# algbio/founderblockgraphs

Hardware: AMD Instinct MI355X
Metric: MSA columns segmented/sec (higher is better)
Workload: dtype u32

## Files before the change

founderblockgraphs_amd/csrc/ctx.hip:

```cpp
#include "fbg_internal.h"
#include <chrono>
#include <stdarg.h>
#include <stdio.h>
#include <ctype.h>
#include <string.h>
#include <algorithm>
#include <atomic>
#include <thread>
#include <vector>

static std::string g_global_err;

int fbg_fail(fbg_ctx *ctx, int code, const char *fmt, ...)
{
    char buf[1024];
    va_list ap;
    va_start(ap, fmt);
    vsnprintf(buf, sizeof(buf), fmt, ap);
    va_end(ap);
    if (ctx) ctx->err = buf; else g_global_err = buf;
    return code;
}

int fbg_reserve(fbg_ctx *ctx, DevBuf &b, size_t bytes, std::vector<DevBuf *> *owner, bool accounted)
// ... 167 lines not shown
    {"gapped_rank", &FbgOptions::gapped_rank},
    {"part_tricks_off", &FbgOptions::part_tricks_off},
    {"msd_sample_bins", &FbgOptions::msd_sample_bins},
    {"msd_min_force", &FbgOptions::msd_min_force},
    {"msd_probe", &FbgOptions::msd_probe},
    {"msd_xcd", &FbgOptions::msd_xcd},
    {"rank_no_lean", &FbgOptions::rank_no_lean},
    {"no_stream_upload", &FbgOptions::no_stream_upload},
    {"span_scan", &FbgOptions::span_scan},
    {"span_key_flags", &FbgOptions::span_key_flags},
    {"span_slow_split", &FbgOptions::span_slow_split},
    {"poison", &FbgOptions::poison},
    {"dpw_matrix", &FbgOptions::dpw_matrix},
    {"dp_chain1", &FbgOptions::dp_chain1},
    {"msd_ext", &FbgOptions::msd_ext},
};

struct InfoKey { const char *name; int64_t (*get)(const fbg_ctx &); };
static const InfoKey g_info_keys[] = {
    {"grs_threshold", [](const fbg_ctx &c) -> int64_t { return c.grs_t; }},
    {"grs_redone", [](const fbg_ctx &c) -> int64_t { return (int64_t)c.grs_redone; }},
    {"dp_kind", [](const fbg_ctx &c) -> int64_t { return c.dp_kind; }},
    {"msd_decline", [](const fbg_ctx &c) -> int64_t { return c.diag.msd_decline; }},
    {"pass1_ahead", [](const fbg_ctx &c) -> int64_t { return c.diag.pass1_ahead; }},
    {"ext_pairs", [](const fbg_ctx &c) -> int64_t { return c.diag.ext_pairs; }},
    {"text_pairs", [](const fbg_ctx &c) -> int64_t { return c.diag.text_pairs; }},
    {"rank_lean_used", [](const fbg_ctx &c) -> int64_t { return c.diag.rank_lean_used; }},
    {"rank_lean_launched", [](const fbg_ctx &c) -> int64_t { return c.diag.rank_lean_launched; }},
    {"pairs_rb", [](const fbg_ctx &c) -> int64_t { return c.diag.pairs_rb; }},
    {"key_b", [](const fbg_ctx &c) -> int64_t { return c.key_b; }},
    {"key_K", [](const fbg_ctx &c) -> int64_t { return c.key_K; }},
    {"key_packed", [](const fbg_ctx &c) -> int64_t { return c.key_packed; }},
    {"key_compact", [](const fbg_ctx &c) -> int64_t { return c.key_compact; }},
    {"alloc_calls", [](const fbg_ctx &c) -> int64_t { return (int64_t)c.alloc_calls; }},
    {"alloc_us", [](const fbg_ctx &c) -> int64_t { return (int64_t)c.alloc_us; }},
    {"span_decline", [](const fbg_ctx &c) -> int64_t { return c.diag.sp_decline; }},
    {"span_key_flags_used", [](const fbg_ctx &c) -> int64_t { return c.ix.index_valid && c.ix.spanned() && c.ix.sp_key_flags_sorted; }},
    {"span_scan_used", [](const fbg_ctx &c) -> int64_t { return c.ix.index_valid && c.ix.spanned(); }},
    {"span_scan_work", [](const fbg_ctx &c) -> int64_t { return (int64_t)c.sp_work; }},
    {"span_groups", [](const fbg_ctx &c) -> int64_t { return (int64_t)c.sp_G; }},
    {"span_odd_groups", [](const fbg_ctx &c) -> int64_t { return (int64_t)c.sp_n_odd[0] + c.sp_n_odd[1] + c.sp_n_odd[2] + c.sp_n_odd[3]; }},
    {"span_irregular", [](const fbg_ctx &c) -> int64_t { return (int64_t)c.sp_n_irr; }},
// ... 519 lines not shown
```

founderblockgraphs_amd/csrc/fbg_internal.h:

```cpp
#pragma once
#include <cstring>
#include <cstdlib>
#include <hip/hip_runtime.h>
#include <stdint.h>
#include <string>
#include <vector>
#include "../../include/fbg_hip.h"

#define FBG_WAVE 64

struct DevBuf {
    void *p = nullptr;
    size_t cap = 0;
    bool listed = false;
    template <class T> T *as() const { return reinterpret_cast<T *>(p); }
};

struct Stager {
    void *base = nullptr;
    size_t slot_bytes = 0;
    int nslots = 0;
    hipEvent_t *ev = nullptr;
    hipStream_t stream = nullptr;
};

struct StageTimer {
    hipEvent_t start = nullptr, stop = nullptr;
    bool recorded = false;
    int launches = 0;
};

struct FbgOptions {
    int64_t no_ranked = 0, no_packed = 0, force_wide = 0, full_keys = 0, no_msd_sort = 0, msd_min = -1, bp_min = -1,
            record_scatter = 0, lcp_text = 0, no_aux_stream = 0, rank_no_threshold = 0, dp_literal = 0, dp_wave = 0,
            dp_safe_window = 0, dp_tile = 0, pure_scan = 0, gapped_rank = 0, part_tricks_off = 0, msd_sample_bins = 0, msd_min_force = 0, msd_probe = 0, msd_xcd = -1, rank_no_lean = 0, no_stream_upload = 0,
            span_scan = 0, span_key_flags = 0, span_slow_split = 0, poison = 0, dpw_matrix = 0, dp_chain1 = 0, msd_ext = 1;
};

enum class IndexKind { none, record, ranked, gapped, span };

struct IndexState {
    bool index_valid = false;
    IndexKind kind = IndexKind::none;
    bool ranked() const { return kind == IndexKind::ranked; }
    bool granked() const { return kind == IndexKind::gapped || kind == IndexKind::span; }
    bool spanned() const { return kind == IndexKind::span; }
    uint32_t *sa_ptr = nullptr;
    uint64_t *rk_keys = nullptr;
    int rk_b = 0, rk_key_bits = 0, rk_K = 0;
    int rk_layout = 0, rk_pb = 0;
    bool grs_flagged = false;
// ... 4 lines not shown
    uint32_t n_exc = 0;
    bool part_active = false;
    bool gpart = false;
    int part = 0, nparts = 1;
    uint64_t part_count = 0;
    uint64_t part_T = 0;
    uint32_t part_gmin = 0;
};

struct BuildDiag {
    int64_t msd_decline = -1;
    int pass1_ahead = 0;
    int64_t ext_pairs = -1, text_pairs = -1;
    int rank_lean_launched = 0;
    int rank_lean_used = 0;
    int pairs_rb = -1;
    int sp_decline = 0;
};

struct SortExtras {
    const uint64_t *ebits = nullptr;
    const uint32_t *payload = nullptr;
    bool key_flags = false;
};

struct MsdPlan;
struct fbg_ctx {
    int device = 0;
    FbgOptions opt;
    std::string err;
// ... 17 lines not shown
    bool allow_wide = false;
    uint32_t mp = 0;
    DevBuf text;
    DevBuf pos, tot;
    DevBuf segtab;
    DevBuf colT;
    DevBuf gwin_rows;

    const uint8_t *up_host = nullptr;
    hipStream_t up_stream = nullptr;
    hipEvent_t up_ev[9] = {};
    bool pre_pass1 = false;
    uint64_t pre_symbols[4] = {0, 0, 0, 0};
    MsdPlan *pre_plan = nullptr;
    uint64_t pre_tiles = 0;

    IndexState ix;
    BuildDiag diag;
    int key_b = -1, key_K = -1, key_packed = -1, key_compact = -1;
    int dp_kind = -1;
    bool grs_skip = false;
    bool cells_built = false;
    uint64_t held_bytes = 0;
    uint64_t alloc_calls = 0, alloc_us = 0;
    std::vector<DevBuf *> bufs;

    DevBuf prow;
    DevBuf igrow;
    DevBuf rec;
    DevBuf xlist;
// ... 40 lines not shown
    do {                             \
        int rc_ = (expr);            \
        if (rc_ != FBG_OK) return rc_; \
    } while (0)

int fbg_reserve(fbg_ctx *ctx, DevBuf &b, size_t bytes, std::vector<DevBuf *> *owner, bool accounted);
inline int fbg_reserve(fbg_ctx *ctx, DevBuf &b, size_t bytes) { return fbg_reserve(ctx, b, bytes, &ctx->bufs, true); }
void fbg_release(fbg_ctx *ctx, DevBuf &b);
void fbg_release_all(fbg_ctx *ctx, std::vector<DevBuf *> &bufs);
void fbg_index_reset(fbg_ctx *ctx);
int fbg_upload(fbg_ctx *ctx, void *d_dst, const void *h_src, size_t bytes);
int fbg_download(fbg_ctx *ctx, void *h_dst, const void *d_src, size_t bytes);
int fbg_stage_begin(fbg_ctx *ctx, int stage);
int fbg_stage_end(fbg_ctx *ctx, int stage, int launches);

#define FBG_SLOTS_PAIRS 0
#define FBG_SLOTS_PACKED 1
#define FBG_SLOTS_WIDE 2
struct KeyGeom {
    int b = 0, K = 0, key_bits = 0;
    bool compact = false, packed = false;
    bool wide = false;
    int pb = 0;
    const uint8_t *d_code = nullptr;
};

inline void fbg_remember_slots(fbg_ctx *ctx, uint64_t *keys, uint32_t *vals, int layout, const KeyGeom &g)
{
    ctx->ix.rk_keys = keys; ctx->ix.sa_ptr = vals; ctx->ix.rk_layout = layout; ctx->ix.rk_pb = g.pb;
    ctx->ix.rk_b = g.b; ctx->ix.rk_key_bits = g.key_bits; ctx->ix.rk_K = g.K;
// ... 25 lines not shown
bool fbg_span_key_flags(fbg_ctx *ctx, KeyGeom &g);
int fbg_span_prepare(fbg_ctx *ctx, const KeyGeom &g, const SortExtras &x, int *launches);
int fbg_span_try(fbg_ctx *ctx, uint64_t *keys, uint32_t *vals, const KeyGeom &g, int *done);
int fbg_span_rescan(fbg_ctx *ctx, int disable_tricks, int *ok);
int fbg_build_cell_tables(fbg_ctx *ctx);
int fbg_key_setup(fbg_ctx *ctx, bool compact, KeyGeom *g, int *launches);
int fbg_rank_part_classify(fbg_ctx *ctx, uint64_t *keys, uint32_t *vals, uint64_t count, const KeyGeom &g, int pre_ok,
                           uint8_t *d_blob, int *ok);
int fbg_rank_part_runs(fbg_ctx *ctx, const uint8_t *d_blobs, uint32_t *d_gmax, int *ok);
int fbg_rank_part_unfilled(fbg_ctx *ctx, uint64_t *unfilled);
int fbg_rank_part_rescan(fbg_ctx *ctx);
int fbg_part_sort(fbg_ctx *ctx, int part, int nparts, uint8_t *d_blob, int *ok);
int fbg_msd_sort(fbg_ctx *ctx, const KeyGeom &g, uint64_t **sorted, int *ok, int *launches);
int fbg_msd_pre_begin(fbg_ctx *ctx, int *ok);
int fbg_msd_pre_pass1(fbg_ctx *ctx, uint64_t avail);
bool fbg_msd_pre_geom(fbg_ctx *ctx, KeyGeom *g);
void fbg_msd_pre_free(fbg_ctx *ctx);
int fbg_msd_sort_part(fbg_ctx *ctx, const KeyGeom &g, uint64_t lo, uint64_t hi, int nohi, int nparts, uint64_t out_offset,
                      uint64_t *count, int *ok, int *launches);
int fbg_sample_sort_pairs(fbg_ctx *ctx, const KeyGeom &g, const SortExtras &x, int *ok, int *launches);
int fbg_scan_columns(fbg_ctx *ctx, uint64_t x0, uint64_t x1, int mode, int disable_tricks,
                     uint64_t *d_out);
int fbg_dp_minmax(fbg_ctx *ctx, const uint64_t *d_f, uint64_t n, uint64_t *d_boundaries,
                  uint64_t *count_out, uint64_t *d_mml, uint64_t *d_bt);
int fbg_dp_repeatfree(fbg_ctx *ctx, const uint64_t *d_v, uint64_t n, uint64_t *d_s,
                      uint64_t *d_prev, uint64_t *d_boundaries, uint64_t *count_out);
int fbg_gapped_v_from_f(fbg_ctx *ctx, const uint64_t *d_f, uint64_t n, uint64_t *d_v);
int fbg_dp_gapped(fbg_ctx *ctx, const uint64_t *d_v, uint64_t n, uint64_t *d_s, uint64_t *d_prev,
                  uint64_t *d_boundaries, uint64_t *count_out);

// ... 11 lines not shown
```

founderblockgraphs_amd/csrc/msd_keys.h:

```cpp
#pragma once
#include <stdint.h>

#define MSD_SEP 0x80
#define MSD_ITEMS 8

template <int TILE>
__device__ __forceinline__ void msd_fetch_raw(const uint8_t *__restrict__ T, uint64_t N, uint64_t base, uint64_t &raw, uint64_t &raw2)
{
    const uint64_t p = base + threadIdx.x * 8;
    raw = p < N + 56 ? *reinterpret_cast<const uint64_t *>(T + p) : 0ull;
    raw2 = 0;
    if (threadIdx.x < 8) {
        const uint64_t q = base + TILE + threadIdx.x * 8;
        raw2 = q < N + 56 ? *reinterpret_cast<const uint64_t *>(T + q) : 0ull;
    }
}
template <int TILE, bool FULL = false>
__device__ __forceinline__ void msd_store_tile(uint8_t *tile, const uint8_t *cd, uint64_t N, uint64_t base, uint64_t raw, uint64_t raw2)
{
    const int k8 = threadIdx.x * 8;
    const uint64_t p = base + k8;
    uint64_t codes = 0;
#pragma unroll
    for (int j = 0; j < 8; j++) {
// ... 9 lines not shown
        for (int j = 0; j < 8; j++) {
            const uint32_t c = (FULL || q + j < N) ? cd[(raw2 >> (8 * j)) & 255u] : (uint32_t)MSD_SEP;
            codes2 |= (uint64_t)c << (8 * j);
        }
        *reinterpret_cast<uint64_t *>(tile + kk) = codes2;
    }
}
template <int TILE, bool FULL = false>
__device__ __forceinline__ void msd_load_tile(uint8_t *tile, const uint8_t *cd, const uint8_t *__restrict__ T, uint64_t N, uint64_t base)
{
    uint64_t raw, raw2;
    msd_fetch_raw<TILE>(T, N, base, raw, raw2);
    msd_store_tile<TILE, FULL>(tile, cd, N, base, raw, raw2);
}

__device__ __forceinline__ void msd_build_keys(const uint8_t *tile, int t0, int b, int K, uint64_t *w)
{
    bool slow = true;
    if (b == 2 && K + MSD_ITEMS - 1 <= 32) {
        uint64_t P = 0, any = 0;
#pragma unroll
        for (int q = 0; q < 4; q++) {
            const uint64_t x = *reinterpret_cast<const uint64_t *>(tile + t0 + 8 * q);
            any |= x;
            const uint32_t lo = (uint32_t)x & 0x03030303u, hi = (uint32_t)(x >> 32) & 0x03030303u;
            const uint32_t g = (((lo * 0x40100401u) >> 24) << 8) | ((hi * 0x40100401u) >> 24);
            P |= (uint64_t)g << (48 - 16 * q);
        }
        slow = (any & 0x8080808080808080ull) != 0;
#pragma unroll
// ... 31 lines not shown
```

founderblockgraphs_amd/csrc/msd_sort.hip:

```cpp
#include "fbg_internal.h"
#include "msd_keys.h"
#include <rocprim/rocprim.hpp>
#include <algorithm>
#include <cmath>

#define MSD_DIG 9
#define MSD_NB (1 << MSD_DIG)
#define MSD_THREADS 1024
#define MSD_TILE (MSD_THREADS * MSD_ITEMS)
#define MSD_TILE_BITS 13
#define MSD_XSYM 4
#define MSD_XBITS 8
static_assert(MSD_TILE == 1 << MSD_TILE_BITS, "tile size");
#define MSD_FN_THREADS 512
#define MSD_FN_CAP 4096
#define MSD_FN_ITEMS (MSD_FN_CAP / MSD_FN_THREADS)
#define MSD_FN_BITS 11
#define MSD_FN_BINS (1 << MSD_FN_BITS)
#define MSD_BIG_THREADS 1024
#define MSD_BIG_CAP 16384
#define MSD_ARENA (1u << 20)

struct MsdArgs {
    const uint8_t *T;
    uint64_t N;
    const uint8_t *code;
    int b, K, pb, kb;
    int xb;
    uint8_t *ext;
    uint64_t *buf1;
    uint64_t cap1;
    int xs;
    uint64_t segcap;
    unsigned long long *count1;
    const uint32_t *tile_start;
    uint64_t tile0;
    uint32_t tiles2, tiles2_x;
    uint64_t *buf2;
    uint32_t *count2;
    const unsigned long long *off;
    uint64_t *out;
// ... 13 lines not shown
#pragma unroll
    for (int d = 1; d < 64; d <<= 1) { const uint32_t o = __shfl_up(inc, d, 64); if ((int)lane >= d) inc += o; }
    if (lane == 63) wsum[wv] = inc;
    __syncthreads();
    uint32_t pre = 0;
    for (uint32_t q = 0; q < wv; q++) pre += wsum[q];
    if (threadIdx.x < MSD_NB) {
        loff[threadIdx.x] = pre + inc - c;
        unsigned long long g = 0;
        if (c) g = wide_cursor ? atomicAdd(cursor_d, (unsigned long long)c) : (unsigned long long)atomicAdd(cursor32_d, c);
        gdelta[threadIdx.x] = (uint32_t)g - (pre + inc - c);
    }
    __syncthreads();
}

template <bool FULL, bool EXT>
__device__ __forceinline__ void msd_pack_split_body(const MsdArgs &a, uint64_t *buf, const uint8_t *cd, uint32_t *cnt, uint32_t *loff, uint32_t *gdelta,
                                                    uint32_t *wsum)
{
    uint8_t *tile = reinterpret_cast<uint8_t *>(buf);
    const int b = a.b, K = a.K;
    const uint64_t base = ((uint64_t)blockIdx.x + a.tile0) * MSD_TILE;
    msd_load_tile<MSD_TILE, FULL>(tile, cd, a.T, a.N, base);
    __syncthreads();
    const int t0 = threadIdx.x * MSD_ITEMS;
    uint64_t w[MSD_ITEMS];
    msd_build_keys(tile, t0, b, EXT ? K + MSD_XSYM : K, w);
    __syncthreads();
    uint32_t rk[MSD_ITEMS];
    const int dshift = a.kb + (EXT ? MSD_XBITS : 0) - MSD_DIG;
#pragma unroll
    for (int i = 0; i < MSD_ITEMS; i++) {
        const uint64_t p = base + t0 + i;
        const bool ok = FULL || p < a.N;
        rk[i] = ok ? atomicAdd(&cnt[(uint32_t)(w[i] >> dshift)], 1u) : 0xffffffffu;
        w[i] = EXT ? (w[i] << MSD_TILE_BITS) | (uint64_t)(t0 + i) : (w[i] << a.pb) | p;
    }
    __syncthreads();
// ... 11 lines not shown
#pragma unroll
    for (int r = 0; r < MSD_ITEMS; r++) {
        const uint32_t j = threadIdx.x + r * MSD_THREADS;
        if (FULL || j < have) {
            uint64_t x = buf[j];
            const uint32_t d = (uint32_t)(x >> wshift);
            if (EXT) x = (((x >> MSD_TILE_BITS) & kmask) << a.pb) | (base + (x & (MSD_TILE - 1)));
            const uint32_t at = j + gdelta[d];
            if (at < a.segcap) obase[(uint64_t)d * a.cap1 + at] = x;
            else over = true;
        }
    }
    if (over) atomicOr(a.flag, 2ull);
}

template <bool EXT>
__global__ __launch_bounds__(MSD_THREADS) void k_msd_pack_split(MsdArgs a)
{
    __shared__ uint64_t buf[MSD_TILE];
    __shared__ uint8_t cd[256];
    __shared__ uint32_t cnt[MSD_NB], loff[MSD_NB];
    __shared__ uint32_t gdelta[MSD_NB];
    __shared__ uint32_t wsum[MSD_THREADS / 64];
    if (threadIdx.x < 256) cd[threadIdx.x] = a.code[threadIdx.x];
    if (threadIdx.x < MSD_NB) cnt[threadIdx.x] = 0;
    __syncthreads();
    msd_pack_split_body<false, EXT>(a, buf, cd, cnt, loff, gdelta, wsum);
}

static void msd_launch_pass1(const MsdArgs &a, unsigned tiles, hipStream_t st)
{
    if (a.xb) hipLaunchKernelGGL(k_msd_pack_split<true>, dim3(tiles), dim3(MSD_THREADS), 0, st, a);
    else hipLaunchKernelGGL(k_msd_pack_split<false>, dim3(tiles), dim3(MSD_THREADS), 0, st, a);
}

__global__ __launch_bounds__(1024) void k_msd_tiles(const unsigned long long *__restrict__ count1, uint64_t segcap, uint32_t nseg,
                                                    uint32_t *__restrict__ tile_start, unsigned long long *__restrict__ flag)
{
    __shared__ uint32_t wsum[16];
    const uint32_t lane = threadIdx.x & 63, wv = threadIdx.x >> 6;
    uint32_t t[4], tot = 0;
#pragma unroll
    for (int q = 0; q < 4; q++) {
        const uint32_t s = threadIdx.x * 4 + q;
        t[q] = 0;
        if (s < nseg) {
            const unsigned long long c = count1[s] < segcap ? count1[s] : segcap;
            if (count1[s] > segcap) atomicOr(flag, 4ull);
// ... 310 lines not shown
    const uint64_t cap1 = (N / MSD_NB + N / (4 * MSD_NB) + 65536) & ~127ull;
    const uint64_t nsub = (uint64_t)MSD_NB * MSD_NB;
    if (N / nsub + N / (32 * nsub) + 64 > MSD_FN_CAP) return FBG_OK;
    FBG_TRY(fbg_reserve(ctx, ctx->keysA, (size_t)MSD_NB * cap1 * 8));
    FBG_TRY(fbg_reserve(ctx, ctx->keysB, (size_t)nsub * MSD_FN_CAP * 8));
    const uint32_t nseg = MSD_NB * (uint32_t)xs;
    FBG_TRY(fbg_reserve(ctx, ctx->dp_a, (size_t)nseg * 8 + ((size_t)nseg + 1) * 4 + 64));
    FBG_TRY(fbg_reserve(ctx, ctx->dp_b, nsub * 4));
    FBG_TRY(fbg_reserve(ctx, ctx->dp_c, (nsub + 1) * 8));
    FBG_TRY(fbg_reserve(ctx, ctx->dp_d, (size_t)MSD_ARENA * 4 * 2));
    FBG_TRY(fbg_reserve(ctx, ctx->dp_e, (size_t)MSD_ARENA * 8 * 2));
    const bool ext = ctx->opt.msd_ext != 0 && g.b == 2 && g.key_bits + MSD_XBITS + MSD_TILE_BITS <= 64 && g.K + MSD_XSYM + MSD_ITEMS - 1 <= 64;
    if (ext) FBG_TRY(fbg_reserve(ctx, ctx->msd_ext, (size_t)N));
    unsigned long long *flag = ctx->scalars.as<unsigned long long>() + 100;
    MsdArgs &a = p->a;
    a.T = ctx->text.as<uint8_t>(); a.N = N; a.code = g.d_code; a.b = g.b; a.K = g.K; a.pb = g.pb; a.kb = g.key_bits;
    a.xb = ext ? MSD_XBITS : 0; a.ext = ext ? ctx->msd_ext.as<uint8_t>() : nullptr;
    a.buf1 = ctx->keysA.as<uint64_t>(); a.cap1 = cap1; a.xs = xs; a.segcap = cap1 / xs;
    a.tile0 = 0; a.tiles2 = 0; a.tiles2_x = 0;
    a.count1 = ctx->dp_a.as<unsigned long long>();
    p->tile_start = reinterpret_cast<uint32_t *>(ctx->dp_a.as<uint8_t>() + (size_t)nseg * 8);
    a.tile_start = p->tile_start;
    a.buf2 = ctx->keysB.as<uint64_t>();
    a.count2 = ctx->dp_b.as<uint32_t>();
    p->off = ctx->dp_c.as<unsigned long long>();
    a.off = p->off;
    a.out = ctx->keysA.as<uint64_t>();
    a.flag = flag;
    a.arena_sb = ctx->dp_d.as<uint32_t>(); a.arena_w = ctx->dp_e.as<uint64_t>(); a.arena_count = flag + 1; a.arena_cap = MSD_ARENA;
    p->g = g; p->nsub = nsub; p->nseg = nseg; p->rest = rest; p->fbits = fbits; p->xcd = xcd; p->flag = flag;
    FBG_HIP_TRY(ctx, hipMemsetAsync(flag, 0, 16, st));
// ... 21 lines not shown
    return FBG_OK;
}

int fbg_msd_pre_pass1(fbg_ctx *ctx, uint64_t avail)
{
    MsdArgs a = ctx->pre_plan->a;
    const uint64_t N = a.N;
    const uint64_t upto = avail >= N ? (N + MSD_TILE - 1) / MSD_TILE : (avail >= 64 ? (avail - 64) / MSD_TILE : 0);
    if (upto <= ctx->pre_tiles) return FBG_OK;
    a.tile0 = ctx->pre_tiles;
    msd_launch_pass1(a, (unsigned)(upto - ctx->pre_tiles), ctx->stream);
    ctx->pre_tiles = upto;
    return FBG_OK;
}

void fbg_msd_pre_free(fbg_ctx *ctx)
{
    delete ctx->pre_plan;
    ctx->pre_plan = nullptr;
}

static bool msd_plan_current(const fbg_ctx *ctx, const MsdPlan &p)
{
    const MsdArgs &a = p.a;
    return a.T == ctx->text.p && a.code == ctx->small.as<uint8_t>() + 2048 && a.buf1 == ctx->keysA.p && a.out == ctx->keysA.p &&
           a.buf2 == ctx->keysB.p && a.count1 == ctx->dp_a.p && (const void *)p.tile_start == ctx->dp_a.as<uint8_t>() + (size_t)p.nseg * 8 &&
           a.count2 == ctx->dp_b.p && p.off == ctx->dp_c.p && a.arena_sb == ctx->dp_d.p && a.arena_w == ctx->dp_e.p &&
           p.flag == ctx->scalars.as<unsigned long long>() + 100 && (!a.xb || a.ext == ctx->msd_ext.p);
}

bool fbg_msd_pre_geom(fbg_ctx *ctx, KeyGeom *g)
{
    if (!ctx->pre_pass1) return false;
    if (!msd_plan_current(ctx, *ctx->pre_plan)) { ctx->pre_pass1 = false; return false; }
    *g = ctx->pre_plan->g;
    fbg_note_key_geom(ctx, *g);
    return true;
}

int fbg_msd_sort(fbg_ctx *ctx, const KeyGeom &g, uint64_t **sorted, int *ok, int *launches)
{
    *ok = 0;
    ctx->diag.msd_decline = 1;
    ctx->ix.msd_ext_valid = false;
    const uint64_t N = ctx->N;
    hipStream_t st = ctx->stream;
    MsdPlan plan;
    const bool ahead = ctx->pre_pass1 && msd_plan_current(ctx, *ctx->pre_plan);
    ctx->pre_pass1 = false;
    ctx->diag.pass1_ahead = ahead ? 1 : 0;
    if (ahead) plan = *ctx->pre_plan;
    else {
        int good = 0;
        FBG_TRY(msd_plan(ctx, g, &plan, &good));
        if (!good) return FBG_OK;
    }
    MsdArgs &a = plan.a;
    const uint64_t nsub = plan.nsub;
    const uint32_t nseg = plan.nseg;
    const int rest = plan.rest, fbits = plan.fbits, xcd = plan.xcd;
    uint32_t *tile_start = plan.tile_start;
    unsigned long long *off = plan.off, *flag = plan.flag;
    if (!ahead) {
        FBG_TRY(fbg_stage_begin(ctx, FBG_STAGE_SORT_PASS1));
        msd_launch_pass1(a, fbg_blocks(N, MSD_TILE), st);
        FBG_TRY(fbg_stage_end(ctx, FBG_STAGE_SORT_PASS1, 1));
    }
    hipLaunchKernelGGL(k_msd_tiles, dim3(1), dim3(1024), 0, st, a.count1, a.segcap, nseg, tile_start, flag);
    uint32_t tiles2 = 0;
    unsigned long long h_flag = 0;
    FBG_HIP_TRY(ctx, hipMemcpyAsync(&tiles2, tile_start + nseg, 4, hipMemcpyDeviceToHost, st));
    FBG_HIP_TRY(ctx, hipMemcpyAsync(&h_flag, flag, 8, hipMemcpyDeviceToHost, st));
    FBG_HIP_TRY(ctx, hipStreamSynchronize(st));
    *launches += 2;
    ctx->diag.msd_decline = (int64_t)h_flag;
    if (h_flag != 0 || tiles2 == 0) return FBG_OK;
    a.tiles2 = tiles2;
    a.tiles2_x = (xcd & 1) ? (tiles2 + 7) / 8 : 0;
    const unsigned grid2 = a.tiles2_x ? 8 * a.tiles2_x : tiles2;
    FBG_TRY(fbg_stage_begin(ctx, FBG_STAGE_SORT_PASS2));
    hipLaunchKernelGGL(k_msd_split, dim3(grid2), dim3(MSD_THREADS), 0, st, a);
    FBG_TRY(fbg_stage_end(ctx, FBG_STAGE_SORT_PASS2, 1));
    unsigned long long *wide = reinterpret_cast<unsigned long long *>(ctx->keysA.p);
    hipLaunchKernelGGL(k_msd_widen, dim3(fbg_blocks(nsub, 256)), dim3(256), 0, st, a.count2, wide, nsub);
    {
        size_t bytes = 0;
        hipError_t e = rocprim::exclusive_scan(nullptr, bytes, wide, off, 0ull, (size_t)nsub, rocprim::plus<unsigned long long>(), st);
        if (e != hipSuccess) return fbg_fail(ctx, FBG_ERR_HIP, "rocprim scan size query: %s", hipGetErrorString(e));
        FBG_TRY(fbg_reserve(ctx, ctx->tmp, bytes));
// ... 40 lines not shown
```

founderblockgraphs_amd/csrc/suffix_sort.hip:

```cpp
#include "fbg_internal.h"
#include "text_cmp.h"
#include <rocprim/rocprim.hpp>
#include <utility>
#include <cmath>

#define SS_THREADS 256

using fbg_sort_config = rocprim::radix_sort_config<
    rocprim::default_config, rocprim::default_config,
    rocprim::radix_sort_onesweep_config<rocprim::kernel_config<512, 32>, rocprim::kernel_config<1024, 8>, 9,
                                        rocprim::block_radix_rank_algorithm::match>>;

#define PK_ITEMS 8
#define FBG_SEP 0x80
struct PackArgs {
    const uint8_t *T;
    uint64_t N;
    const uint8_t *code;
    int b, K, pb;
    uint64_t *keys;
    uint32_t *vals;
    uint64_t lo, hi, cap;
    int nohi;
    unsigned long long *counter;
// ... 600 lines not shown
    return FBG_OK;
}

int fbg_key_setup(fbg_ctx *ctx, bool compact, KeyGeom *g, int *launches)
{
    const uint64_t N = ctx->N;
    hipStream_t st = ctx->stream;
    uint8_t *d_code = ctx->small.as<uint8_t>() + 2048;
    const uint64_t *hist = ctx->byte_hist;
    if (hist[0] != 1)
        return fbg_fail(ctx, FBG_ERR_INVALID, "the MSA contains a NUL byte; the text needs a unique 0 sentinel");
    int below = 0, real = 0;
    for (int c = 1; c < 256; c++)
        if (hist[c] && c != '#') { real++; if (c < '#') below++; }
    compact = compact && below == 0 && real >= 1 && real < FBG_SEP;
    uint8_t code[256];
    int sigma = 0;
    if (compact) {
        for (int c = 0; c < 256; c++) {
            if (c == 0 || c == '#') { code[c] = FBG_SEP; continue; }
            code[c] = (uint8_t)sigma;
            if (hist[c]) sigma++;
        }
    } else {
        for (int c = 0; c < 256; c++) { code[c] = (uint8_t)sigma; if (hist[c]) sigma++; }
    }
    int b = 1;
    while ((1 << b) < sigma) b++;
    double H = 0;
    for (int c = 1; c < 256; c++)
        if (hist[c] && !(compact && c == '#')) { const double q = (double)hist[c] / (double)N; H -= q * log2(q); }
// ... 9 lines not shown
    if (N >= (1ull << 32) || (compact && ctx->opt.force_wide)) {
        if (!compact) return fbg_fail(ctx, FBG_ERR_TOO_LARGE, "text length %llu needs >32-bit positions", (unsigned long long)N);
        int pb = 1;
        while ((1ull << (32 + pb)) < N) pb++;
        g->wide = true; g->pb = pb;
        if (K > (64 - pb) / b) K = (64 - pb) / b;
    } else if (compact && !ctx->opt.no_packed) {
        int pb = 1;
        while ((1ull << pb) < N) pb++;
        const int Kroom = (64 - pb) / b;
        const int Kmin = (int)ceil((log2((double)N) + 3.2) / H);
        if (Kroom >= Kmin) { g->packed = true; g->pb = pb; if (K > Kroom) K = Kroom; }
    }
    g->b = b; g->K = K; g->key_bits = K * b; g->d_code = d_code;
    fbg_note_key_geom(ctx, *g);
    FBG_HIP_TRY(ctx, hipMemcpyAsync(d_code, code, 256, hipMemcpyHostToDevice, st));
    FBG_HIP_TRY(ctx, hipStreamSynchronize(st));
    *launches += 1;
    return FBG_OK;
}

static int sort_slots(fbg_ctx *ctx, const KeyGeom &g, bool key_flags, uint64_t count, uint64_t out_offset)
{
    hipStream_t st = ctx->stream;
    uint64_t *ka = ctx->keysA.as<uint64_t>(), *kb = ctx->keysB.as<uint64_t>() + out_offset;
    if (g.packed) {
        unsigned lo = (unsigned)g.pb;
        const unsigned hi = (unsigned)(g.pb + g.key_bits);
        if (hi == 64 && count < (1u << 23)) lo = 0;
        return with_tmp(ctx, [&](void *tmp, size_t &bytes) {
            return rocprim::radix_sort_keys<fbg_sort_config>(tmp, bytes, ka, kb, (size_t)count, lo, hi, st);
// ... 23 lines not shown
    hipLaunchKernelGGL(k_sample_keys, dim3(fbg_blocks(S, 256)), dim3(256), 0, st, ctx->text.as<uint8_t>(), N, g.d_code, g.b, g.K,
                       g.compact ? 1 : 0, stride, S, smp);
    FBG_TRY(with_tmp(ctx, [&](void *tmp, size_t &bytes) {
        return rocprim::radix_sort_keys(tmp, bytes, smp, srt, (size_t)S, 0u, (unsigned)g.key_bits, st);
    }));
    hipLaunchKernelGGL(k_count_equal_neighbours, dim3(fbg_blocks(S, 256)), dim3(256), 0, st, srt, S, d_count);
    unsigned long long twins = 0;
    FBG_HIP_TRY(ctx, hipMemcpyAsync(&twins, d_count, 8, hipMemcpyDeviceToHost, st));
    FBG_HIP_TRY(ctx, hipStreamSynchronize(st));
    *launches += 3;
    const double est = (double)twins * (double)N / ((double)S * (double)S);
    *similar = est > 0.5;
    return FBG_OK;
}

int fbg_suffix_sort(fbg_ctx *ctx)
{
    const uint64_t N = ctx->N;
    hipStream_t st = ctx->stream;
    FBG_TRY(fbg_stage_begin(ctx, FBG_STAGE_SUFFIX_SORT));
    int launches = 0;
    const uint8_t *T = ctx->text.as<uint8_t>();
    KeyGeom g;
    SortExtras x;

    if (ctx->gapfree && !ctx->have_ignore && !ctx->opt.no_ranked) {
        if (!fbg_msd_pre_geom(ctx, &g)) FBG_TRY(fbg_key_setup(ctx, true, &g, &launches));
    }
    if (ctx->gapfree && !ctx->have_ignore && !ctx->opt.no_ranked && g.compact) {
        bool similar = false;
        FBG_TRY(sample_says_similar(ctx, g, &similar, &launches));
        uint64_t *sorted = nullptr;
        int msd_ok = 0;
        FBG_TRY(fbg_msd_sort(ctx, g, &sorted, &msd_ok, &launches));
        if (!msd_ok) {
            FBG_TRY(fbg_reserve(ctx, ctx->keysA, N * 8));
            FBG_TRY(fbg_reserve(ctx, ctx->keysB, N * 8));
            if (!g.packed) {
                FBG_TRY(fbg_reserve(ctx, ctx->valsA, N * 4));
                FBG_TRY(fbg_reserve(ctx, ctx->valsB, N * 4));
            }
            PackArgs pa;
            pa.T = T; pa.N = N; pa.code = g.d_code; pa.b = g.b; pa.K = g.K; pa.pb = g.pb;
            pa.keys = ctx->keysA.as<uint64_t>(); pa.vals = ctx->valsA.as<uint32_t>();
            pa.lo = pa.hi = pa.cap = 0; pa.nohi = 1; pa.counter = nullptr;
            launch_pack(ctx, g, false, pa, x);
            launches++;
            FBG_TRY(sort_slots(ctx, g, false, N, 0));
            sorted = ctx->keysB.as<uint64_t>();
// ... 299 lines not shown
```

founderblockgraphs_amd/csrc/text_build.hip:

```cpp
#include "fbg_internal.h"

#define TB_THREADS 256
#define TB_ITEMS 8
#define TB_CHUNK (TB_THREADS * TB_ITEMS)

__device__ __forceinline__ uint32_t wave_incl_scan(uint32_t v)
{
    const int lane = threadIdx.x & 63;
#pragma unroll
    for (int d = 1; d < 64; d <<= 1) {
        uint32_t o = __shfl_up(v, d, 64);
        if (lane >= d) v += o;
    }
    return v;
}

__device__ __forceinline__ uint32_t block_excl_scan(uint32_t v, uint32_t *total, uint32_t *lds4)
{
    const int lane = threadIdx.x & 63, w = threadIdx.x >> 6;
    uint32_t inc = wave_incl_scan(v);
    if (lane == 63) lds4[w] = inc;
    __syncthreads();
    uint32_t base = 0, tot = 0;
#pragma unroll
// ... 155 lines not shown

__global__ void k_row_offsets(const uint32_t *__restrict__ tot, uint64_t m, uint32_t *__restrict__ pos,
                              unsigned long long *__restrict__ scalars)
{
    if (blockIdx.x != 0 || threadIdx.x >= 64) return;
    const uint64_t per = (m + 63) / 64, lo = min(m, (uint64_t)threadIdx.x * per), hi = min(m, lo + per);
    unsigned long long mine = 0;
    for (uint64_t i = lo; i < hi; i++) mine += (unsigned long long)tot[i] + 1;
    unsigned long long inc = mine;
    for (int d = 1; d < 64; d <<= 1) { const unsigned long long o = __shfl_up(inc, d, 64); if ((int)threadIdx.x >= d) inc += o; }
    unsigned long long s = inc - mine;
    for (uint64_t i = lo; i < hi; i++) { pos[i] = (uint32_t)s; s += (unsigned long long)tot[i] + 1; }
    if (threadIdx.x == 63) scalars[2] = inc + 1;
}

__global__ void k_seg_offsets(const uint32_t *__restrict__ segcnt, uint64_t m, uint32_t nseg, uint32_t *__restrict__ segoff)
{
    const uint64_t i = (uint64_t)blockIdx.x * blockDim.x + threadIdx.x;
    if (i >= m) return;
    uint32_t run = 0;
    for (uint32_t q = 0; q < nseg; q++) { segoff[i * nseg + q] = run; run += segcnt[i * nseg + q]; }
}

template <bool GAPPED, bool REVERSED>
__global__ __launch_bounds__(TB_THREADS) void k_write_text(const uint8_t *__restrict__ msa, uint64_t n,
                                                           const uint32_t *__restrict__ pos,
                                                           const uint32_t *__restrict__ tot,
                                                           uint8_t *__restrict__ T, uint32_t *__restrict__ prow,
                                                           uint32_t *__restrict__ colT, const uint32_t *__restrict__ segoff,
                                                           uint16_t *__restrict__ winrow)
// ... 168 lines not shown
    ctx->have_ignore = ignore_len > 0;
    ctx->cells_built = false;
    memset(ctx->ignore_tab, 0, sizeof(ctx->ignore_tab));
    if (ctx->have_ignore) {
        for (uint64_t k = 0; k < ignore_len; k++) ctx->ignore_tab[ignore[k]] = 1;
        FBG_HIP_TRY(ctx, hipMemcpyAsync(ctx->small.as<uint8_t>(), ctx->ignore_tab, 256, hipMemcpyHostToDevice, st));
    }
    unsigned long long *sc = ctx->scalars.as<unsigned long long>();
    unsigned long long *d_hist = reinterpret_cast<unsigned long long *>(ctx->small.as<uint8_t>() + 4096);
    FBG_HIP_TRY(ctx, hipMemsetAsync(d_hist, 0, 2048, st));
    FBG_HIP_TRY(ctx, hipMemsetAsync(ctx->tot.p, 0, m * 4, st));
    const unsigned nseg = (unsigned)((n + RC_SEG - 1) / RC_SEG);
    FBG_TRY(fbg_reserve(ctx, ctx->segtab, (size_t)m * nseg * 4 * 3));
    uint32_t *segcnt = ctx->segtab.as<uint32_t>(), *segoff = segcnt + (size_t)m * nseg;
    const bool fused = !ctx->reversed && n % 8 == 0 && ((uintptr_t)ctx->d_msa & 7) == 0 && m * (n + 1) + 1 < (1ull << 40);
    if (fused) FBG_TRY(fbg_reserve(ctx, ctx->text, m * (n + 1) + 1 + 64));
    const uint8_t *up = ctx->up_host;
    ctx->up_host = nullptr;
    ctx->pre_pass1 = false;
    if (up && fused && m >= 16) {
        constexpr int CHUNKS = 8;
        if (!ctx->up_stream) {
            FBG_HIP_TRY(ctx, hipStreamCreateWithFlags(&ctx->up_stream, hipStreamNonBlocking));
            for (auto &e : ctx->up_ev) FBG_HIP_TRY(ctx, hipEventCreateWithFlags(&e, hipEventDisableTiming));
        }
        uint8_t *d_msa = ctx->msa_own.as<uint8_t>();
        FBG_HIP_TRY(ctx, hipEventRecord(ctx->up_ev[CHUNKS], st));
        FBG_HIP_TRY(ctx, hipStreamWaitEvent(ctx->up_stream, ctx->up_ev[CHUNKS], 0));
        uint64_t r0s[CHUNKS + 1];
        for (int c = 0; c <= CHUNKS; c++) r0s[c] = m * c / CHUNKS;
        for (int c = 0; c < CHUNKS; c++) {
            FBG_HIP_TRY(ctx, hipMemcpyAsync(d_msa + r0s[c] * n, up + r0s[c] * n, (r0s[c + 1] - r0s[c]) * n, hipMemcpyHostToDevice, ctx->up_stream));
            FBG_HIP_TRY(ctx, hipEventRecord(ctx->up_ev[c], ctx->up_stream));
        }
// ... 12 lines not shown
                    ctx->byte_hist['-'] = 0; ctx->byte_hist['#'] += m; ctx->byte_hist[0] += 1;
                    ctx->N = m * (n + 1) + 1;
                    ctx->gapfree = true;
                    FBG_HIP_TRY(ctx, hipMemsetAsync(ctx->text.as<uint8_t>() + ctx->N - 1, 0, 65, st));
                    int ok = 0;
                    FBG_TRY(fbg_msd_pre_begin(ctx, &ok));
                    pre = ok != 0;
                }
            }
            if (pre) FBG_TRY(fbg_msd_pre_pass1(ctx, c + 1 < CHUNKS ? r0s[c + 1] * (n + 1) : ctx->N));
        }
        ctx->pre_pass1 = pre;
        launches += CHUNKS - 1;
    } else {
        if (up) FBG_TRY(fbg_upload(ctx, ctx->msa_own.p, up, m * n));
        hipLaunchKernelGGL(k_row_count, dim3(nseg, (unsigned)m), dim3(TB_THREADS), 0, st, ctx->d_msa,
                           n, (const uint8_t *)nullptr, ctx->tot.as<uint32_t>(), sc, d_hist, segcnt, fused ? ctx->text.as<uint8_t>() : (uint8_t *)nullptr);
    }
    hipLaunchKernelGGL(k_row_offsets, dim3(1), dim3(64), 0, st, ctx->tot.as<uint32_t>(), m,
                       ctx->pos.as<uint32_t>(), sc);
    launches += 2;
    unsigned long long h[3];
    FBG_HIP_TRY(ctx, hipMemcpyAsync(h, sc, sizeof(h), hipMemcpyDeviceToHost, st));
    FBG_HIP_TRY(ctx, hipMemcpyAsync(ctx->byte_hist, d_hist, 256 * sizeof(uint64_t), hipMemcpyDeviceToHost, st));
    FBG_HIP_TRY(ctx, hipStreamSynchronize(st));
    ctx->byte_hist['-'] = 0;
    ctx->byte_hist['#'] += m;
    ctx->byte_hist[0] += 1;
    ctx->gapfree = h[0] == 0;
    ctx->N = h[2];
// ... 104 lines not shown
```

Measured before the change: 60.98 million.

## Build MSD pass-1 keys directly from MSA, writing text speculatively

```diff
diff --git a/founderblockgraphs_amd/csrc/ctx.hip b/founderblockgraphs_amd/csrc/ctx.hip
--- a/founderblockgraphs_amd/csrc/ctx.hip
+++ b/founderblockgraphs_amd/csrc/ctx.hip
@@ -205,6 +205,8 @@
     {"dpw_matrix", &FbgOptions::dpw_matrix},
     {"dp_chain1", &FbgOptions::dp_chain1},
     {"msd_ext", &FbgOptions::msd_ext},
+    {"msd_from_msa", &FbgOptions::msd_from_msa},
+    {"msa_sample_rows", &FbgOptions::msa_sample_rows},
 };
 
 struct InfoKey { const char *name; int64_t (*get)(const fbg_ctx &); };
@@ -217,6 +219,7 @@
     {"ext_pairs", [](const fbg_ctx &c) -> int64_t { return c.diag.ext_pairs; }},
     {"text_pairs", [](const fbg_ctx &c) -> int64_t { return c.diag.text_pairs; }},
     {"rank_lean_used", [](const fbg_ctx &c) -> int64_t { return c.diag.rank_lean_used; }},
+    {"text_fused_used", [](const fbg_ctx &c) -> int64_t { return c.diag.text_fused_used; }},
     {"rank_lean_launched", [](const fbg_ctx &c) -> int64_t { return c.diag.rank_lean_launched; }},
     {"pairs_rb", [](const fbg_ctx &c) -> int64_t { return c.diag.pairs_rb; }},
     {"key_b", [](const fbg_ctx &c) -> int64_t { return c.key_b; }},
diff --git a/founderblockgraphs_amd/csrc/fbg_internal.h b/founderblockgraphs_amd/csrc/fbg_internal.h
--- a/founderblockgraphs_amd/csrc/fbg_internal.h
+++ b/founderblockgraphs_amd/csrc/fbg_internal.h
@@ -34,7 +34,7 @@
     int64_t no_ranked = 0, no_packed = 0, force_wide = 0, full_keys = 0, no_msd_sort = 0, msd_min = -1, bp_min = -1,
             record_scatter = 0, lcp_text = 0, no_aux_stream = 0, rank_no_threshold = 0, dp_literal = 0, dp_wave = 0,
             dp_safe_window = 0, dp_tile = 0, pure_scan = 0, gapped_rank = 0, part_tricks_off = 0, msd_sample_bins = 0, msd_min_force = 0, msd_probe = 0, msd_xcd = -1, rank_no_lean = 0, no_stream_upload = 0,
-            span_scan = 0, span_key_flags = 0, span_slow_split = 0, poison = 0, dpw_matrix = 0, dp_chain1 = 0, msd_ext = 1;
+            span_scan = 0, span_key_flags = 0, span_slow_split = 0, poison = 0, dpw_matrix = 0, dp_chain1 = 0, msd_ext = 1, msd_from_msa = 1, msa_sample_rows = 0;
 };
 
 enum class IndexKind { none, record, ranked, gapped, span };
@@ -69,6 +69,7 @@
     int64_t ext_pairs = -1, text_pairs = -1;
     int rank_lean_launched = 0;
     int rank_lean_used = 0;
+    int text_fused_used = 0;
     int pairs_rb = -1;
     int sp_decline = 0;
 };
@@ -116,6 +117,8 @@
     uint64_t pre_symbols[4] = {0, 0, 0, 0};
     MsdPlan *pre_plan = nullptr;
     uint64_t pre_tiles = 0;
+    bool pre_msa = false;
+    bool no_pre_msa = false;
 
     IndexState ix;
     BuildDiag diag;
@@ -186,6 +189,7 @@
 int fbg_stage_begin(fbg_ctx *ctx, int stage);
 int fbg_stage_end(fbg_ctx *ctx, int stage, int launches);
 
+#define FBG_CODE_UNPROMISED 0xC0
 #define FBG_SLOTS_PAIRS 0
 #define FBG_SLOTS_PACKED 1
 #define FBG_SLOTS_WIDE 2
@@ -241,6 +245,7 @@
 int fbg_msd_sort(fbg_ctx *ctx, const KeyGeom &g, uint64_t **sorted, int *ok, int *launches);
 int fbg_msd_pre_begin(fbg_ctx *ctx, int *ok);
 int fbg_msd_pre_pass1(fbg_ctx *ctx, uint64_t avail);
+int fbg_msd_pre_from_msa(fbg_ctx *ctx);
 bool fbg_msd_pre_geom(fbg_ctx *ctx, KeyGeom *g);
 void fbg_msd_pre_free(fbg_ctx *ctx);
 int fbg_msd_sort_part(fbg_ctx *ctx, const KeyGeom &g, uint64_t lo, uint64_t hi, int nohi, int nparts, uint64_t out_offset,
diff --git a/founderblockgraphs_amd/csrc/msd_keys.h b/founderblockgraphs_amd/csrc/msd_keys.h
--- a/founderblockgraphs_amd/csrc/msd_keys.h
+++ b/founderblockgraphs_amd/csrc/msd_keys.h
@@ -47,6 +47,48 @@
     msd_store_tile<TILE, FULL>(tile, cd, N, base, raw, raw2);
 }
 
+#define MSD_UNPROMISED 0xC0
+template <int TILE>
+__device__ __forceinline__ bool msd_msa_eight(uint8_t *tile, const uint8_t *cd, const uint8_t *__restrict__ msa, uint32_t n, uint64_t N,
+                                              uint64_t base, uint32_t row0, uint32_t col0, uint32_t off, uint8_t *__restrict__ Tw, bool store)
+{
+    typedef uint64_t u64_unaligned __attribute__((aligned(1)));
+    const uint32_t L = n + 1;
+    uint32_t r = row0, q = col0 + off;
+    if (L <= (uint32_t)TILE + 72) { r += q / L; q %= L; }
+    else if (q >= L) { q -= L; r++; }
+    const uint64_t p = base + off;
+    uint64_t raw = 0, codes = 0;
+    if (q + 8 <= n && p + 8 < N) {
+        raw = *reinterpret_cast<const u64_unaligned *>(msa + (p - r));
+#pragma unroll
+        for (int j = 0; j < 8; j++) codes |= (uint64_t)cd[(raw >> (8 * j)) & 255u] << (8 * j);
+    } else {
+        for (int j = 0; j < 8; j++) {
+            uint32_t c = MSD_SEP, byte = 0;
+            if (p + j < N - 1) {
+                uint32_t rj = r, qj = q + j;
+                while (qj >= L) { qj -= L; rj++; }
+                byte = '#';
+                if (qj != n) { byte = msa[p + j - rj]; c = cd[byte]; }
+            }
+            raw |= (uint64_t)byte << (8 * j);
+            codes |= (uint64_t)c << (8 * j);
+        }
+    }
+    *reinterpret_cast<uint64_t *>(tile + off) = codes;
+    if (store && p < N + 64) *reinterpret_cast<uint64_t *>(Tw + p) = raw;
+    return (codes & (codes << 1) & 0x8080808080808080ull) != 0;
+}
+template <int TILE>
+__device__ __forceinline__ bool msd_load_tile_msa(uint8_t *tile, const uint8_t *cd, const uint8_t *__restrict__ msa, uint32_t n, uint64_t N,
+                                                  uint64_t base, uint32_t row0, uint32_t col0, uint8_t *__restrict__ Tw)
+{
+    bool bad = msd_msa_eight<TILE>(tile, cd, msa, n, N, base, row0, col0, threadIdx.x * 8, Tw, true);
+    if (threadIdx.x < 8) bad |= msd_msa_eight<TILE>(tile, cd, msa, n, N, base, row0, col0, TILE + threadIdx.x * 8, Tw, base + TILE >= N);
+    return bad;
+}
+
 __device__ __forceinline__ void msd_build_keys(const uint8_t *tile, int t0, int b, int K, uint64_t *w)
 {
     bool slow = true;
diff --git a/founderblockgraphs_amd/csrc/msd_sort.hip b/founderblockgraphs_amd/csrc/msd_sort.hip
--- a/founderblockgraphs_amd/csrc/msd_sort.hip
+++ b/founderblockgraphs_amd/csrc/msd_sort.hip
@@ -3,6 +3,7 @@
 #include <rocprim/rocprim.hpp>
 #include <algorithm>
 #include <cmath>
+#include <vector>
 
 #define MSD_DIG 9
 #define MSD_NB (1 << MSD_DIG)
@@ -25,6 +26,9 @@
     const uint8_t *T;
     uint64_t N;
     const uint8_t *code;
+    const uint8_t *msa = nullptr;
+    uint32_t msa_n = 0;
+    uint8_t *Tw = nullptr;
     int b, K, pb, kb;
     int xb;
     uint8_t *ext;
@@ -68,14 +72,17 @@
     __syncthreads();
 }
 
-template <bool FULL, bool EXT>
+template <bool FULL, bool EXT, bool MSA>
 __device__ __forceinline__ void msd_pack_split_body(const MsdArgs &a, uint64_t *buf, const uint8_t *cd, uint32_t *cnt, uint32_t *loff, uint32_t *gdelta,
-                                                    uint32_t *wsum)
+                                                    uint32_t *wsum, const uint32_t *rc)
 {
     uint8_t *tile = reinterpret_cast<uint8_t *>(buf);
     const int b = a.b, K = a.K;
     const uint64_t base = ((uint64_t)blockIdx.x + a.tile0) * MSD_TILE;
-    msd_load_tile<MSD_TILE, FULL>(tile, cd, a.T, a.N, base);
+    if (MSA) {
+        if (msd_load_tile_msa<MSD_TILE>(tile, cd, a.msa, a.msa_n, a.N, base, rc[0], rc[1], a.Tw) &&
+            __ffsll((long long)__ballot(1)) - 1 == (int)(threadIdx.x & 63)) atomicOr(a.flag, 32ull);
+    } else msd_load_tile<MSD_TILE, FULL>(tile, cd, a.T, a.N, base);
     __syncthreads();
     const int t0 = threadIdx.x * MSD_ITEMS;
     uint64_t w[MSD_ITEMS];
@@ -117,7 +124,7 @@
     if (over) atomicOr(a.flag, 2ull);
 }
 
-template <bool EXT>
+template <bool EXT, bool MSA>
 __global__ __launch_bounds__(MSD_THREADS) void k_msd_pack_split(MsdArgs a)
 {
     __shared__ uint64_t buf[MSD_TILE];
@@ -125,16 +132,25 @@
     __shared__ uint32_t cnt[MSD_NB], loff[MSD_NB];
     __shared__ uint32_t gdelta[MSD_NB];
     __shared__ uint32_t wsum[MSD_THREADS / 64];
-    if (threadIdx.x < 256) cd[threadIdx.x] = a.code[threadIdx.x];
+    __shared__ uint32_t rc[2];
+    if (threadIdx.x < 256) cd[threadIdx.x] = a.code[threadIdx.x + (MSA ? 256 : 0)];
     if (threadIdx.x < MSD_NB) cnt[threadIdx.x] = 0;
-    __syncthreads();
-    msd_pack_split_body<false, EXT>(a, buf, cd, cnt, loff, gdelta, wsum);
+    if (MSA && threadIdx.x == MSD_NB) {
+        const uint32_t base = (uint32_t)(((uint64_t)blockIdx.x + a.tile0) * MSD_TILE), L = a.msa_n + 1;
+        rc[0] = base / L;
+        rc[1] = base % L;
+    }
+    __syncthreads();
+    msd_pack_split_body<false, EXT, MSA>(a, buf, cd, cnt, loff, gdelta, wsum, rc);
 }
 
 static void msd_launch_pass1(const MsdArgs &a, unsigned tiles, hipStream_t st)
 {
-    if (a.xb) hipLaunchKernelGGL(k_msd_pack_split<true>, dim3(tiles), dim3(MSD_THREADS), 0, st, a);
-    else hipLaunchKernelGGL(k_msd_pack_split<false>, dim3(tiles), dim3(MSD_THREADS), 0, st, a);
+    if (a.msa) {
+        if (a.xb) hipLaunchKernelGGL((k_msd_pack_split<true, true>), dim3(tiles), dim3(MSD_THREADS), 0, st, a);
+        else hipLaunchKernelGGL((k_msd_pack_split<false, true>), dim3(tiles), dim3(MSD_THREADS), 0, st, a);
+    } else if (a.xb) hipLaunchKernelGGL((k_msd_pack_split<true, false>), dim3(tiles), dim3(MSD_THREADS), 0, st, a);
+    else hipLaunchKernelGGL((k_msd_pack_split<false, false>), dim3(tiles), dim3(MSD_THREADS), 0, st, a);
 }
 
 __global__ __launch_bounds__(1024) void k_msd_tiles(const unsigned long long *__restrict__ count1, uint64_t segcap, uint32_t nseg,
@@ -475,7 +491,7 @@
     if (ext) FBG_TRY(fbg_reserve(ctx, ctx->msd_ext, (size_t)N));
     unsigned long long *flag = ctx->scalars.as<unsigned long long>() + 100;
     MsdArgs &a = p->a;
-    a.T = ctx->text.as<uint8_t>(); a.N = N; a.code = g.d_code; a.b = g.b; a.K = g.K; a.pb = g.pb; a.kb = g.key_bits;
+    a.T = ctx->text.as<uint8_t>(); a.N = N; a.code = g.d_code; a.msa = nullptr; a.msa_n = 0; a.Tw = nullptr; a.b = g.b; a.K = g.K; a.pb = g.pb; a.kb = g.key_bits;
     a.xb = ext ? MSD_XBITS : 0; a.ext = ext ? ctx->msd_ext.as<uint8_t>() : nullptr;
     a.buf1 = ctx->keysA.as<uint64_t>(); a.cap1 = cap1; a.xs = xs; a.segcap = cap1 / xs;
     a.tile0 = 0; a.tiles2 = 0; a.tiles2_x = 0;
@@ -527,6 +543,15 @@
     return FBG_OK;
 }
 
+int fbg_msd_pre_from_msa(fbg_ctx *ctx)
+{
+    MsdArgs &a = ctx->pre_plan->a;
+    a.msa = ctx->d_msa; a.msa_n = (uint32_t)ctx->n; a.Tw = ctx->text.as<uint8_t>();
+    FBG_TRY(fbg_stage_begin(ctx, FBG_STAGE_SORT_PASS1));
+    FBG_TRY(fbg_msd_pre_pass1(ctx, a.N));
+    return fbg_stage_end(ctx, FBG_STAGE_SORT_PASS1, 1);
+}
+
 void fbg_msd_pre_free(fbg_ctx *ctx)
 {
     delete ctx->pre_plan;
@@ -548,6 +573,28 @@
     if (!msd_plan_current(ctx, *ctx->pre_plan)) { ctx->pre_pass1 = false; return false; }
     *g = ctx->pre_plan->g;
     fbg_note_key_geom(ctx, *g);
+    return true;
+}
+
+static bool msd_hist_from_counts(fbg_ctx *ctx, const KeyGeom &g, const unsigned long long *count1, int xs)
+{
+    if (!g.compact || g.b > MSD_DIG) return false;
+    uint64_t by_code[1 << MSD_DIG] = {0}, total = 0;
+    for (uint32_t d = 0; d < MSD_NB; d++)
+        for (int x = 0; x < xs; x++) { by_code[d >> (MSD_DIG - g.b)] += count1[d * xs + x]; total += count1[d * xs + x]; }
+    if (total != ctx->N || by_code[0] < ctx->m + 1) return false;
+    by_code[0] -= ctx->m + 1;
+    uint64_t hist[256] = {0};
+    int code = 0;
+    for (int c = 1; c < 256; c++) {
+        if (c == '#' || !((ctx->pre_symbols[c >> 6] >> (c & 63)) & 1ull)) continue;
+        if (code >= (1 << g.b) || by_code[code] == 0) return false;
+        hist[c] = by_code[code++];
+    }
+    for (; code < (1 << g.b); code++) if (by_code[code]) return false;
+    hist['#'] = ctx->m;
+    hist[0] = 1;
+    memcpy(ctx->byte_hist, hist, sizeof(hist));
     return true;
 }
 
@@ -561,13 +608,14 @@
     MsdPlan plan;
     const bool ahead = ctx->pre_pass1 && msd_plan_current(ctx, *ctx->pre_plan);
     ctx->pre_pass1 = false;
-    ctx->diag.pass1_ahead = ahead ? 1 : 0;
     if (ahead) plan = *ctx->pre_plan;
     else {
         int good = 0;
         FBG_TRY(msd_plan(ctx, g, &plan, &good));
         if (!good) return FBG_OK;
     }
+    const bool from_msa = ahead && plan.a.msa != nullptr;
+    ctx->diag.pass1_ahead = ahead && !from_msa ? 1 : 0;
     MsdArgs &a = plan.a;
     const uint64_t nsub = plan.nsub;
     const uint32_t nseg = plan.nseg;
@@ -584,8 +632,14 @@
     unsigned long long h_flag = 0;
     FBG_HIP_TRY(ctx, hipMemcpyAsync(&tiles2, tile_start + nseg, 4, hipMemcpyDeviceToHost, st));
     FBG_HIP_TRY(ctx, hipMemcpyAsync(&h_flag, flag, 8, hipMemcpyDeviceToHost, st));
+    std::vector<unsigned long long> h_count1(from_msa ? nseg : 0);
+    if (from_msa) FBG_HIP_TRY(ctx, hipMemcpyAsync(h_count1.data(), a.count1, (size_t)nseg * 8, hipMemcpyDeviceToHost, st));
     FBG_HIP_TRY(ctx, hipStreamSynchronize(st));
     *launches += 2;
+    if (from_msa) {
+        if ((h_flag & 32ull) || !msd_hist_from_counts(ctx, plan.g, h_count1.data(), a.xs)) { ctx->diag.msd_decline = 32; return FBG_OK; }
+        ctx->diag.text_fused_used = 1;
+    }
     ctx->diag.msd_decline = (int64_t)h_flag;
     if (h_flag != 0 || tiles2 == 0) return FBG_OK;
     a.tiles2 = tiles2;
diff --git a/founderblockgraphs_amd/csrc/suffix_sort.hip b/founderblockgraphs_amd/csrc/suffix_sort.hip
--- a/founderblockgraphs_amd/csrc/suffix_sort.hip
+++ b/founderblockgraphs_amd/csrc/suffix_sort.hip
@@ -638,7 +638,7 @@
     for (int c = 1; c < 256; c++)
         if (hist[c] && c != '#') { real++; if (c < '#') below++; }
     compact = compact && below == 0 && real >= 1 && real < FBG_SEP;
-    uint8_t code[256];
+    uint8_t code[512];
     int sigma = 0;
     if (compact) {
         for (int c = 0; c < 256; c++) {
@@ -678,7 +678,8 @@
     }
     g->b = b; g->K = K; g->key_bits = K * b; g->d_code = d_code;
     fbg_note_key_geom(ctx, *g);
-    FBG_HIP_TRY(ctx, hipMemcpyAsync(d_code, code, 256, hipMemcpyHostToDevice, st));
+    for (int c = 0; c < 256; c++) code[256 + c] = (c == 0 || c == '#' || c == '-' || !hist[c]) ? (uint8_t)FBG_CODE_UNPROMISED : code[c];
+    FBG_HIP_TRY(ctx, hipMemcpyAsync(d_code, code, 512, hipMemcpyHostToDevice, st));
     FBG_HIP_TRY(ctx, hipStreamSynchronize(st));
     *launches += 1;
     return FBG_OK;
@@ -732,6 +733,16 @@
     return FBG_OK;
 }
 
+static int suffix_sort_again(fbg_ctx *ctx)
+{
+    ctx->pre_pass1 = false;
+    ctx->no_pre_msa = true;
+    const int rc = fbg_build_text(ctx, nullptr, 0);
+    ctx->no_pre_msa = false;
+    FBG_TRY(rc);
+    return fbg_suffix_sort(ctx);
+}
+
 int fbg_suffix_sort(fbg_ctx *ctx)
 {
     const uint64_t N = ctx->N;
@@ -741,9 +752,14 @@
     const uint8_t *T = ctx->text.as<uint8_t>();
     KeyGeom g;
     SortExtras x;
+    const bool spec = ctx->pre_msa;
+    ctx->pre_msa = false;
 
     if (ctx->gapfree && !ctx->have_ignore && !ctx->opt.no_ranked) {
-        if (!fbg_msd_pre_geom(ctx, &g)) FBG_TRY(fbg_key_setup(ctx, true, &g, &launches));
+        if (!fbg_msd_pre_geom(ctx, &g)) {
+            if (spec) return suffix_sort_again(ctx);
+            FBG_TRY(fbg_key_setup(ctx, true, &g, &launches));
+        }
     }
     if (ctx->gapfree && !ctx->have_ignore && !ctx->opt.no_ranked && g.compact) {
         bool similar = false;
@@ -751,6 +767,7 @@
         uint64_t *sorted = nullptr;
         int msd_ok = 0;
         FBG_TRY(fbg_msd_sort(ctx, g, &sorted, &msd_ok, &launches));
+        if (spec && !ctx->diag.text_fused_used) return suffix_sort_again(ctx);
         if (!msd_ok) {
             FBG_TRY(fbg_reserve(ctx, ctx->keysA, N * 8));
             FBG_TRY(fbg_reserve(ctx, ctx->keysB, N * 8));
diff --git a/founderblockgraphs_amd/csrc/text_build.hip b/founderblockgraphs_amd/csrc/text_build.hip
--- a/founderblockgraphs_amd/csrc/text_build.hip
+++ b/founderblockgraphs_amd/csrc/text_build.hip
@@ -1,4 +1,5 @@
 #include "fbg_internal.h"
+#include <algorithm>
 
 #define TB_THREADS 256
 #define TB_ITEMS 8
@@ -193,6 +194,16 @@
     if (threadIdx.x == 63) scalars[2] = inc + 1;
 }
 
+__global__ void k_gapfree_tables(uint64_t m, uint64_t n, uint32_t nseg, uint32_t *__restrict__ tot, uint32_t *__restrict__ pos,
+                                 uint32_t *__restrict__ segcnt)
+{
+    const uint64_t k = (uint64_t)blockIdx.x * blockDim.x + threadIdx.x;
+    if (k >= m * nseg) return;
+    const uint64_t i = k / nseg, q = k % nseg;
+    segcnt[k] = (uint32_t)min((uint64_t)RC_SEG, n - q * RC_SEG);
+    if (q == 0) { tot[i] = (uint32_t)n; pos[i] = (uint32_t)(i * (n + 1)); }
+}
+
 __global__ void k_seg_offsets(const uint32_t *__restrict__ segcnt, uint64_t m, uint32_t nseg, uint32_t *__restrict__ segoff)
 {
     const uint64_t i = (uint64_t)blockIdx.x * blockDim.x + threadIdx.x;
@@ -391,10 +402,11 @@
     FBG_TRY(fbg_reserve(ctx, ctx->segtab, (size_t)m * nseg * 4 * 3));
     uint32_t *segcnt = ctx->segtab.as<uint32_t>(), *segoff = segcnt + (size_t)m * nseg;
     const bool fused = !ctx->reversed && n % 8 == 0 && ((uintptr_t)ctx->d_msa & 7) == 0 && m * (n + 1) + 1 < (1ull << 40);
-    if (fused) FBG_TRY(fbg_reserve(ctx, ctx->text, m * (n + 1) + 1 + 64));
+    if (fused) FBG_TRY(fbg_reserve(ctx, ctx->text, m * (n + 1) + 1 + 72));
     const uint8_t *up = ctx->up_host;
     ctx->up_host = nullptr;
     ctx->pre_pass1 = false;
+    ctx->pre_msa = false;
     if (up && fused && m >= 16) {
         constexpr int CHUNKS = 8;
         if (!ctx->up_stream) {
@@ -437,6 +449,42 @@
         launches += CHUNKS - 1;
     } else {
         if (up) FBG_TRY(fbg_upload(ctx, ctx->msa_own.p, up, m * n));
+        const uint64_t N_gapfree = m * (n + 1) + 1;
+        const uint64_t msd_min = ctx->opt.msd_min >= 0 ? (uint64_t)ctx->opt.msd_min : (1ull << 24);
+        if (ctx->opt.msd_from_msa && !ctx->no_pre_msa && !ctx->allow_wide && !ctx->have_ignore && !ctx->reversed && !ctx->opt.no_ranked &&
+            !ctx->opt.no_msd_sort && N_gapfree < (1ull << 31) && N_gapfree >= msd_min) {
+            const uint64_t R = std::min<uint64_t>(std::min<uint64_t>(m, 65535),
+                                                  ctx->opt.msa_sample_rows > 0 ? (uint64_t)ctx->opt.msa_sample_rows : ((4ull << 20) + n - 1) / n);
+            hipLaunchKernelGGL(k_row_count, dim3(nseg, (unsigned)R), dim3(TB_THREADS), 0, st, ctx->d_msa, n, (const uint8_t *)nullptr,
+                               ctx->tot.as<uint32_t>(), sc, d_hist, segcnt, (uint8_t *)nullptr);
+            unsigned long long h0[1];
+            FBG_HIP_TRY(ctx, hipMemcpyAsync(h0, sc, sizeof(h0), hipMemcpyDeviceToHost, st));
+            FBG_HIP_TRY(ctx, hipMemcpyAsync(ctx->byte_hist, d_hist, 256 * sizeof(uint64_t), hipMemcpyDeviceToHost, st));
+            FBG_HIP_TRY(ctx, hipStreamSynchronize(st));
+            launches++;
+            if (h0[0] == 0 && ctx->byte_hist[0] == 0 && ctx->byte_hist['#'] == 0) {
+                for (int b = 0; b < 256; b++) ctx->byte_hist[b] = ctx->byte_hist[b] * m / R;
+                ctx->byte_hist['-'] = 0; ctx->byte_hist['#'] += m; ctx->byte_hist[0] += 1;
+                ctx->N = N_gapfree;
+                ctx->gapfree = true;
+                ctx->mp = (uint32_t)((m + 63) & ~63ull);
+                FBG_TRY(fbg_reserve(ctx, ctx->text, ctx->N + 72));
+                int ok = 0;
+                FBG_TRY(fbg_msd_pre_begin(ctx, &ok));
+                if (ok) {
+                    hipLaunchKernelGGL(k_gapfree_tables, dim3(fbg_blocks(m * nseg, 256)), dim3(256), 0, st, m, n, nseg, ctx->tot.as<uint32_t>(),
+                                       ctx->pos.as<uint32_t>(), segcnt);
+                    FBG_TRY(fbg_msd_pre_from_msa(ctx));
+                    ctx->pre_pass1 = true;
+                    ctx->pre_msa = true;
+                    FBG_HIP_TRY(ctx, hipGetLastError());
+                    return fbg_stage_end(ctx, FBG_STAGE_TEXT, launches + 2);
+                }
+            }
+            FBG_HIP_TRY(ctx, hipMemsetAsync(ctx->scalars.p, 0, 64 * sizeof(unsigned long long), st));
+            FBG_HIP_TRY(ctx, hipMemsetAsync(d_hist, 0, 2048, st));
+            FBG_HIP_TRY(ctx, hipMemsetAsync(ctx->tot.p, 0, m * 4, st));
+        }
         hipLaunchKernelGGL(k_row_count, dim3(nseg, (unsigned)m), dim3(TB_THREADS), 0, st, ctx->d_msa,
                            n, (const uint8_t *)nullptr, ctx->tot.as<uint32_t>(), sc, d_hist, segcnt, fused ? ctx->text.as<uint8_t>() : (uint8_t *)nullptr);
     }
```

Result: no change. 60.47 million (-0.8%).
